# BienLuky/Rectified-SpaAttn

Hardware: AMD Instinct MI355X
Metric: attention-layer TFLOPs/sec (rectified block-sparse attention, HunyuanVideo seq~120k d=128 bf16) (higher is better)
Workload: dtype bf16; 1 GPU; hunyuan_720p_128f: B=1 H=24 S=115456 (115200 visual + 256 text, 200 valid) D=128, top_k=90, regime=r2 (p_remain=0.0, neighbors=none); heads_per_gpu=24, parallelism=head-shard x1, world_size=1

## Files before the change

### include/rsa.h

```cpp
#ifndef RSA_H_
#define RSA_H_

#include <stddef.h>
#include <stdint.h>

#ifdef __cplusplus
extern "C" {
#endif

#define RSA_BLOCK 128

typedef enum rsa_status {
    RSA_OK = 0,
    RSA_ERR_BAD_ARG = -1,
    RSA_ERR_UNSUPPORTED = -2,
    RSA_ERR_WORKSPACE = -3,
    RSA_ERR_LAUNCH = -4
} rsa_status;

typedef enum rsa_dtype { RSA_BF16 = 0, RSA_FP16 = 1 } rsa_dtype;

typedef struct rsa_layout {
    int32_t B, H, D;
    int32_t S;
// ... 50 lines not shown

int rsa_buffer_bytes(const rsa_layout* lay, size_t sizes[RSA_NUM_BUFFERS], size_t* total);

int rsa_carve_workspace(const rsa_layout* lay, void* ws, size_t ws_bytes, rsa_buffers* out);

int rsa_pool_stats(const rsa_layout* lay, rsa_tensor4 q, rsa_tensor4 k, rsa_tensor4 v, const rsa_buffers* buf,
                   void* stream);

int rsa_pooled_scores(const rsa_layout* lay, rsa_tensor4 k, const rsa_buffers* buf, void* stream);

int rsa_select_mask(const rsa_layout* lay, const uint8_t* neighbor, int top_k, float p_remain,
                    const rsa_buffers* buf, void* stream);

int rsa_compensation(const rsa_layout* lay, const rsa_buffers* buf, void* stream);

int rsa_block_sparse_fwd(const rsa_layout* lay, rsa_tensor4 q, rsa_tensor4 k, rsa_tensor4 v,
                         const rsa_buffers* buf, rsa_out4 out, void* stream);

int rsa_rectified_attention(const rsa_layout* lay, rsa_tensor4 q, rsa_tensor4 k, rsa_tensor4 v,
                            const uint8_t* neighbor, int top_k, float p_remain, void* workspace,
                            size_t workspace_bytes, rsa_out4 out, void* stream);

int rsa_dense_fwd(int B, int H, int Sq, int Sk, int D, int dtype, rsa_tensor4 q, rsa_tensor4 k, rsa_tensor4 v,
                  int q_split, int kv_split, rsa_out4 out, void* stream);
int rsa_dense_causal_fwd(int B, int H, int Sq, int Sk, int D, int dtype, rsa_tensor4 q, rsa_tensor4 k, rsa_tensor4 v,
                         int q_split, int kv_split, rsa_out4 out, void* stream);

#define RSA_MASK_BOOL 1
#define RSA_MASK_ADD_2BYTE 2
#define RSA_MASK_ADD_F32 3
// ... 7 lines not shown
                          uint64_t seed, rsa_out4 out, void* stream);

typedef struct rsa_layout_ex {
    rsa_layout base;
    int32_t block;
    int32_t reserved[3];
} rsa_layout_ex;
int rsa_buffer_bytes_ex(const rsa_layout_ex* lay, size_t sizes[RSA_NUM_BUFFERS], size_t* total);
int rsa_carve_workspace_ex(const rsa_layout_ex* lay, void* ws, size_t ws_bytes, rsa_buffers* out);
int rsa_pool_stats_ex(const rsa_layout_ex* lay, rsa_tensor4 q, rsa_tensor4 k, rsa_tensor4 v, const rsa_buffers* buf,
                      void* stream);
int rsa_pooled_scores_ex(const rsa_layout_ex* lay, rsa_tensor4 k, const rsa_buffers* buf, void* stream);
int rsa_select_mask_ex(const rsa_layout_ex* lay, const uint8_t* neighbor, int top_k, float p_remain,
                       const rsa_buffers* buf, void* stream);
int rsa_compensation_ex(const rsa_layout_ex* lay, const rsa_buffers* buf, void* stream);
int rsa_block_sparse_fwd_ex(const rsa_layout_ex* lay, rsa_tensor4 q, rsa_tensor4 k, rsa_tensor4 v,
                            const rsa_buffers* buf, rsa_out4 out, void* stream);
int rsa_rectified_attention_ex(const rsa_layout_ex* lay, rsa_tensor4 q, rsa_tensor4 k, rsa_tensor4 v,
                               const uint8_t* neighbor, int top_k, float p_remain, void* workspace,
                               size_t workspace_bytes, rsa_out4 out, void* stream);

int rsa_block_mask_to_lists(int B, int H, int NQ, int NK, const uint8_t* mask, int64_t mask_stride_b, int64_t mask_stride_h,
                            int64_t mask_stride_q, uint32_t* bitmask, int32_t* cols, int32_t* counts, void* stream);
int rsa_lists_to_block_mask(int B, int H, int NQ, int NK, const uint32_t* bitmask, uint8_t* mask, void* stream);

int rsa_block_sparse_plain_fwd(int B, int H, int Sq, int Sk, int D, int dtype, int block, int NQ, int NK, int kv_valid,
                               double sm_scale, rsa_tensor4 q, rsa_tensor4 k, rsa_tensor4 v, const int32_t* cols,
                               const int32_t* counts, float* tpart, size_t tpart_bytes, rsa_out4 out, void* stream);

int rsa_select_from_mask(const rsa_layout* lay, const uint8_t* mask, int64_t mask_stride_b, int64_t mask_stride_h,
// ... 110 lines not shown
```

### rectified_spaattn_amd/_core.py

```python
from __future__ import annotations

import ctypes
import math
from dataclasses import dataclass
from typing import Dict, Optional

import torch

from . import _lib
from ._lib import BLOCK, BUFFER_NAMES, RsaBuffers, RsaFp8Operands, RsaLayout, RsaLayoutEx, RsaOut4, RsaTensor4


def check_block(block: int) -> int:
    if block not in _lib.BLOCKS:
        raise NotImplementedError(f"the HIP path is built for block_size_M = block_size_N in {_lib.BLOCKS}, got {block}")
    return int(block)


@dataclass
class LayoutSpec:
    S: int
    NB_total: int
    NBv: int
    n_txt: int
# ... 304 lines not shown
        cb, st = ctypes.byref(self.cb), _stream()
        tk = self.t[1]
        (k2, lay), (k4, _) = self._fn("rsa_pooled_scores"), self._fn("rsa_compensation")
        with torch.cuda.device(self.q.device):
            _lib.check(k2(lay, tk, cb, st), "rsa_pooled_scores")
            if self.mask is not None:
                k3m, _ = self._fn("rsa_select_from_mask")
                _lib.check(k3m(lay, self.mask.data_ptr(), *self.mask_strides, cb, st), "rsa_select_from_mask")
            else:
                k3, _ = self._fn("rsa_select_mask")
                _lib.check(k3(lay, self.nbr.data_ptr() if self.nbr is not None else None, self.top_k,
                              self.p, cb, st), "rsa_select_mask")
            _lib.check(k4(lay, cb, st), "rsa_compensation")

    def select(self):
        self.select_pool()
        self.select_rest()

    def attend(self):
        tq, tk, tv = self.t
        if self.fp8 is not None and self.fp8_pv:
            with torch.cuda.device(self.q.device):
                _lib.check(self.L.rsa_block_sparse_fwd_fp8pv(ctypes.byref(self.lay), tq, tk, ctypes.byref(self.cf),
                                                             ctypes.byref(self.cb), self.o4, _stream()),
                           "rsa_block_sparse_fwd_fp8pv")
            return self.out
        if self.fp8 is not None:
            with torch.cuda.device(self.q.device):
                _lib.check(self.L.rsa_block_sparse_fwd_fp8(ctypes.byref(self.lay), ctypes.byref(self.cf),
                                                           ctypes.byref(self.cb), self.o4, _stream()),
                           "rsa_block_sparse_fwd_fp8")
            return self.out
# ... 199 lines not shown
```

### rectified_spaattn_amd/_lib.py

```python
from __future__ import annotations

import ctypes
import os

import torch

_HERE = os.path.dirname(os.path.abspath(__file__))
LIB_PATH = os.path.join(_HERE, "librsa_hip.so")

RSA_BF16, RSA_FP16 = 0, 1
BLOCK = 128
BLOCKS = (64, 128)
HEADER_VERSION = 601


class RsaError(RuntimeError):
    pass


class RsaLayout(ctypes.Structure):
    _fields_ = [(n, ctypes.c_int32) for n in (
        "B", "H", "D", "S", "NB_total", "NBv", "n_txt", "kv_valid", "pool_valid", "text_end_block",
        "first_frame_blocks", "q_text_valid", "kv_text_valid", "dtype")]

# ... 61 lines not shown
    L.rsa_qk_layernorm_rope.restype = i32
    L.rsa_norm_rope_heads.argtypes = [i32, i32, i32, i32, i32, vp, i64, i64, vp, f32, i32, i32, vp, vp, RsaOut4, vp]
    L.rsa_norm_rope_heads.restype = i32
    L.rsa_rel_l1.argtypes = [vp, vp, i64, i32, vp, vp, vp]
    L.rsa_rel_l1.restype = i32
    L.rsa_set_tuning.argtypes = [ctypes.c_char_p, i32]
    L.rsa_set_tuning.restype = i32
    L.rsa_set_shard_invariant.argtypes = [i32]
    L.rsa_set_shard_invariant.restype = i32
    L.rsa_buffer_bytes.argtypes = [P(RsaLayout), P(sz * NUM_BUFFERS), P(sz)]
    L.rsa_carve_workspace.argtypes = [P(RsaLayout), vp, sz, P(RsaBuffers)]
    L.rsa_pool_stats.argtypes = [P(RsaLayout), RsaTensor4, RsaTensor4, RsaTensor4, P(RsaBuffers), vp]
    L.rsa_pooled_scores.argtypes = [P(RsaLayout), RsaTensor4, P(RsaBuffers), vp]
    L.rsa_select_mask.argtypes = [P(RsaLayout), vp, i32, f32, P(RsaBuffers), vp]
    L.rsa_compensation.argtypes = [P(RsaLayout), P(RsaBuffers), vp]
    L.rsa_block_sparse_fwd.argtypes = [P(RsaLayout), RsaTensor4, RsaTensor4, RsaTensor4, P(RsaBuffers), RsaOut4, vp]
    L.rsa_rectified_attention.argtypes = [P(RsaLayout), RsaTensor4, RsaTensor4, RsaTensor4, vp, i32, f32, vp, sz,
                                          RsaOut4, vp]
    L.rsa_buffer_bytes_ex.argtypes = [P(RsaLayoutEx), P(sz * NUM_BUFFERS), P(sz)]
    L.rsa_carve_workspace_ex.argtypes = [P(RsaLayoutEx), vp, sz, P(RsaBuffers)]
    L.rsa_pool_stats_ex.argtypes = [P(RsaLayoutEx), RsaTensor4, RsaTensor4, RsaTensor4, P(RsaBuffers), vp]
    L.rsa_pooled_scores_ex.argtypes = [P(RsaLayoutEx), RsaTensor4, P(RsaBuffers), vp]
    L.rsa_select_mask_ex.argtypes = [P(RsaLayoutEx), vp, i32, f32, P(RsaBuffers), vp]
    L.rsa_compensation_ex.argtypes = [P(RsaLayoutEx), P(RsaBuffers), vp]
    L.rsa_block_sparse_fwd_ex.argtypes = [P(RsaLayoutEx), RsaTensor4, RsaTensor4, RsaTensor4, P(RsaBuffers), RsaOut4, vp]
    L.rsa_rectified_attention_ex.argtypes = [P(RsaLayoutEx), RsaTensor4, RsaTensor4, RsaTensor4, vp, i32, f32, vp, sz,
                                             RsaOut4, vp]
    L.rsa_estimate_pr_gain_ex.argtypes = [i32] * 6 + [vp] * 9
    L.rsa_block_mask_to_lists.argtypes = [i32] * 4 + [vp, i64, i64, i64, vp, vp, vp, vp]
    L.rsa_lists_to_block_mask.argtypes = [i32] * 4 + [vp, vp, vp]
# ... 50 lines not shown
    L.rsa_ipc_close.argtypes = [vp]
    for name in ("rsa_comm_unique_id", "rsa_comm_create", "rsa_comm_destroy", "rsa_comm_count", "rsa_allgather_heads",
                 "rsa_allgather_heads_p2p", "rsa_ipc_export", "rsa_ipc_open", "rsa_ipc_close", "rsa_ipc_offset",
                 "rsa_p2p_state_alloc", "rsa_p2p_state_free", "rsa_p2p_state_timeout"):
        getattr(L, name).restype = i32
    for name in ("rsa_fp8_operand_bytes", "rsa_carve_fp8_operands", "rsa_quantize_fp8", "rsa_block_sparse_fwd_fp8",
                 "rsa_rectified_attention_fp8", "rsa_rectified_attention_fp8pv", "rsa_pool_stats_fp8", "rsa_dense_fp8_bytes",
                 "rsa_dense_fwd_fp8"):
        getattr(L, name).restype = i32
    for name in ("rsa_buffer_bytes", "rsa_carve_workspace", "rsa_pool_stats", "rsa_pooled_scores",
                 "rsa_select_mask", "rsa_compensation", "rsa_block_sparse_fwd", "rsa_rectified_attention",
                 "rsa_dense_fwd", "rsa_dense_masked_fwd", "rsa_estimate_pr_gain", "rsa_buffer_bytes_ex", "rsa_carve_workspace_ex",
                 "rsa_pool_stats_ex", "rsa_pooled_scores_ex", "rsa_select_mask_ex", "rsa_compensation_ex", "rsa_block_sparse_fwd_ex",
                 "rsa_rectified_attention_ex", "rsa_estimate_pr_gain_ex"):
        getattr(L, name).restype = i32
    for key in ("k5_tsplit", "k3_prefix", "k3_long", "k4_split", "k5_rows256", "k5_static", "k5_w64", "k5_gsync", "k5_gsync_ratio", "k5_text_last", "k5_tail_split"):
        val = os.environ.get("RSA_" + key.upper())
        if val is not None:
            check_rc = L.rsa_set_tuning(key.encode(), int(val))
            if check_rc != 0:
                raise RsaError(f"RSA_{key.upper()} is set but rsa_set_tuning refused it (export RSA_TUNING=1)")
    _lib = L
    return L


EXPORTED = ("rsa_version", "rsa_abi_check", "rsa_buffer_bytes", "rsa_carve_workspace", "rsa_pool_stats", "rsa_pooled_scores",
            "rsa_select_mask", "rsa_compensation", "rsa_block_sparse_fwd", "rsa_rectified_attention",
            "rsa_dense_fwd", "rsa_dense_causal_fwd", "rsa_dense_masked_fwd", "rsa_dense_dropout_fwd", "rsa_estimate_pr_gain", "rsa_status_string", "rsa_last_hip_error", "rsa_set_tuning", "rsa_set_shard_invariant", "rsa_gilbert_mapping",
            "rsa_gilbert_block_neighbors", "rsa_permute_tokens", "rsa_qk_norm_rope", "rsa_qk_layernorm_rope", "rsa_norm_rope_heads", "rsa_fp8_operand_bytes",
            "rsa_carve_fp8_operands", "rsa_quantize_fp8", "rsa_block_sparse_fwd_fp8", "rsa_block_sparse_fwd_fp8pv", "rsa_rectified_attention_fp8", "rsa_rectified_attention_fp8pv",
            "rsa_pool_stats_fp8", "rsa_dense_fp8_bytes", "rsa_dense_fwd_fp8", "rsa_dense_causal_fwd_fp8", "rsa_dense_fwd_fp8pv", "rsa_rel_l1",
            "rsa_comm_unique_id", "rsa_comm_create", "rsa_comm_destroy", "rsa_comm_count", "rsa_allgather_heads",
            "rsa_allgather_heads_p2p", "rsa_p2p_state_bytes", "rsa_p2p_state_alloc", "rsa_p2p_state_free", "rsa_p2p_state_timeout", "rsa_ipc_export", "rsa_ipc_open", "rsa_ipc_close",
            "rsa_ipc_offset", "rsa_buffer_bytes_ex", "rsa_carve_workspace_ex", "rsa_pool_stats_ex", "rsa_pooled_scores_ex",
            "rsa_select_mask_ex", "rsa_compensation_ex", "rsa_block_sparse_fwd_ex", "rsa_rectified_attention_ex", "rsa_estimate_pr_gain_ex",
            "rsa_block_mask_to_lists", "rsa_lists_to_block_mask", "rsa_block_sparse_plain_fwd", "rsa_select_from_mask",
            "rsa_select_from_mask_ex", "rsa_rectified_attention_masked", "rsa_rectified_attention_masked_ex")


def check(status: int, what: str):
    if status == 0:
        return
    msg = f"{what}: {lib().rsa_status_string(status).decode()} (rsa_status {status})"
    if status == -4:
        msg += f": {lib().rsa_last_hip_error().decode()}"
    if status == -2:
        raise AssertionError(msg)
    raise RsaError(msg)
```

### rectified_spaattn_amd/csrc/rsa_attn.hip

```cpp
#include <stdlib.h>

#include <atomic>
#include <mutex>
#include "rsa_attn.h"

static int g_k5_tsplit = 1;
extern int g_rsa_k3_prefix;
extern int g_rsa_k3_long;
extern int g_rsa_k4_split;
extern int g_rsa_k2_dma;
static int g_k5_tail_split = 1;
static int g_k5_text_last = 1;
static int g_shard_invariant = 0;
static int g_k5_gsync_ratio = 2;
int rsa_gsync_ratio() { return g_k5_gsync_ratio; }
static int g_k5_rows256 = 1;
static int g_k5_static = 1;
int rsa_k5_static() { return g_k5_static; }
static int g_k5_gsync = 1;

static int g_k5_w64 = 3;
static bool k5_runs_w64(int D, int blk) { return blk == RSA_BLOCK && ((D == 128 && (g_k5_w64 & 1)) || (D == 64 && (g_k5_w64 & 2))); }

extern "C" int rsa_set_tuning(const char* key, int value) {
    static const bool enabled = [] { const char* e = getenv("RSA_TUNING"); return e && e[0] == '1'; }();
    if (!key) return RSA_ERR_BAD_ARG;
    if (!enabled) return RSA_ERR_UNSUPPORTED;
    if (strcmp(key, "k3_prefix") == 0) { g_rsa_k3_prefix = value; return RSA_OK; }
    if (strcmp(key, "k3_long") == 0) { g_rsa_k3_long = value; return RSA_OK; }
    if (strcmp(key, "k4_split") == 0) { g_rsa_k4_split = value; return RSA_OK; }
    if (strcmp(key, "k2_dma") == 0) { g_rsa_k2_dma = value; return RSA_OK; }
    if (strcmp(key, "k5_static") == 0) { g_k5_static = value; return RSA_OK; }
    if (strcmp(key, "k5_rows256") == 0) { g_k5_rows256 = value; return RSA_OK; }
    if (strcmp(key, "k5_tsplit") == 0) { g_k5_tsplit = value; return RSA_OK; }
    if (strcmp(key, "k5_w64") == 0) { g_k5_w64 = value; return RSA_OK; }
    if (strcmp(key, "k5_gsync") == 0) { g_k5_gsync = value; return RSA_OK; }
    if (strcmp(key, "k5_gsync_ratio") == 0) { g_k5_gsync_ratio = value; return RSA_OK; }
    if (strcmp(key, "k5_text_last") == 0) { g_k5_text_last = value; return RSA_OK; }
    if (strcmp(key, "k5_tail_split") == 0) { g_k5_tail_split = value; return RSA_OK; }
    if (strcmp(key, "fp8_variant") == 0) { rsa_set_fp8_variant(value); return RSA_OK; }
    if (strcmp(key, "fp8_smooth_k") == 0) { rsa_set_fp8_smooth_k(value); return RSA_OK; }
    return RSA_ERR_BAD_ARG;
}

template <typename Tag>
__global__ __launch_bounds__(256) void text_combine_kernel(const float* __restrict__ tpart, unsigned short* out,
// ... 329 lines not shown
                             rsa_tensor4 v, int q_split, int kv_split, rsa_out4 out, void* stream) {
    return dense_fwd(B, H, Sq, Sk, D, dtype, q, k, v, q_split, kv_split, 0, out, stream);
}

extern "C" int rsa_dense_causal_fwd(int B, int H, int Sq, int Sk, int D, int dtype, rsa_tensor4 q, rsa_tensor4 k,
                                    rsa_tensor4 v, int q_split, int kv_split, rsa_out4 out, void* stream) {
    return dense_fwd(B, H, Sq, Sk, D, dtype, q, k, v, q_split, kv_split, 1, out, stream);
}

extern "C" int rsa_rectified_attention(const rsa_layout* l, rsa_tensor4 q, rsa_tensor4 k, rsa_tensor4 v,
                                       const uint8_t* neighbor, int top_k, float p_remain, void* workspace,
                                       size_t workspace_bytes, rsa_out4 out, void* stream) {
    rsa_buffers buf;
    int st = rsa_carve_workspace(l, workspace, workspace_bytes, &buf);
    if (st != RSA_OK) return st;
    if ((st = rsa_pool_stats(l, q, k, v, &buf, stream))) return st;
    if ((st = rsa_pooled_scores(l, k, &buf, stream))) return st;
    if ((st = rsa_select_mask(l, neighbor, top_k, p_remain, &buf, stream))) return st;
    if ((st = rsa_compensation(l, &buf, stream))) return st;
    return rsa_block_sparse_fwd(l, q, k, v, &buf, out, stream);
}

extern "C" int rsa_rectified_attention_ex(const rsa_layout_ex* lx, rsa_tensor4 q, rsa_tensor4 k, rsa_tensor4 v,
                                          const uint8_t* neighbor, int top_k, float p_remain, void* workspace,
                                          size_t workspace_bytes, rsa_out4 out, void* stream) {
    if (!rsa_layout_ex_ok(lx)) return RSA_ERR_BAD_ARG;
    if (lx->block == RSA_BLOCK)
        return rsa_rectified_attention(&lx->base, q, k, v, neighbor, top_k, p_remain, workspace, workspace_bytes, out, stream);
    rsa_buffers buf;
    int st = rsa_carve_workspace_ex(lx, workspace, workspace_bytes, &buf);
    if (st != RSA_OK) return st;
    if ((st = rsa_pool_stats_ex(lx, q, k, v, &buf, stream))) return st;
    if ((st = rsa_pooled_scores_ex(lx, k, &buf, stream))) return st;
    if ((st = rsa_select_mask_ex(lx, neighbor, top_k, p_remain, &buf, stream))) return st;
    if ((st = rsa_compensation_ex(lx, &buf, stream))) return st;
    return rsa_block_sparse_fwd_ex(lx, q, k, v, &buf, out, stream);
}
```

### rectified_spaattn_amd/csrc/rsa_stats.hip

```cpp
#include "rsa_common.h"
#include "rsa_fp8_emit.h"

struct PoolArgs {
    const unsigned short* src[3];
    long sb[3], sh[3], ss[3];
    float* mean[3];
    float* mad[3];
    const float* ext_mean[3];
    int nblk[3];
    int valid[3];
    int H;
    int BH, NB_total;
    Fp8Emit f8;
};

template <int D, typename Tag, bool F8, int BLK = RSA_BLOCK>
__global__ __launch_bounds__(D * 2) void pool_stats_kernel(PoolArgs a) {
    constexpr int NI = BLK / 16;
    constexpr int CH = D / 8;
    constexpr int NTH = 16 * CH;
    constexpr int NW = NTH / 64;
    const int which = F8 ? (int)(blockIdx.x % 3) : (int)blockIdx.z;
    const int blk = F8 ? (int)(blockIdx.x / 3) : (int)blockIdx.x;
    if (blk >= a.nblk[which]) return;
// ... 88 lines not shown
            for (int e = 0; e < 8; ++e) {
                float tot;
                if (NW == 4)
                    tot = (red[0][c * 8 + e] + red[1][c * 8 + e]) +
                          (red[2 % NW][c * 8 + e] + red[3 % NW][c * 8 + e]);
                else
                    tot = red[0][c * 8 + e] + red[1][c * 8 + e];
                r[e] = tot * (1.0f / BLK);
            }
            float4* o = reinterpret_cast<float4*>(a.mad[which] + orow);
            o[0] = make_float4(r[0], r[1], r[2], r[3]);
            o[1] = make_float4(r[4], r[5], r[6], r[7]);
        }
    }
    emit_f8();
}

struct ScoreArgs {
    const float *qbar, *aq, *kbar, *ak;
    const unsigned short* ktxt;
    long ksb, ksh, kss;
    float* scores;
    uint8_t* unrel;
    int NBv, n_txt, NS, D, H, BH;
    int txt0;
};

typedef float k2_f32x16 __attribute__((ext_vector_type(16)));
__device__ __forceinline__ int ncols_of(const ScoreArgs& a, int mode) { return mode == 0 ? a.NBv : a.n_txt; }

// ... 302 lines not shown
            } else if (pos >= len) {
                dl = true;
            }
        }
        c = __shfl(cl, ln, 64);
        count += __shfl(cnt, ln, 64);
        done = __shfl((int)dl, ln, 64) != 0;
        over = __shfl((int)ol, ln, 64) != 0;
    }
    passed = over;
    return count;
}

#define RSA_SEL_CAP 256

template <int KPL, int PASS>
__global__ __launch_bounds__(256) void select_mask_kernel(SelectArgs a) {
    extern __shared__ __attribute__((aligned(16))) unsigned char smem[];
    const int lane = threadIdx.x & 63, wv = threadIdx.x >> 6;
    const long row = (long)blockIdx.x * 4 + wv;
    if (row >= a.rows_total) return;
    if constexpr (PASS == 1) {
        if (a.counts[row] != -1) return;
    }
    const int qblk = (int)(row % a.NBv);
    unsigned char* base = smem + (size_t)wv * a.lds_per_wave;
    float* et = reinterpret_cast<float*>(base);
    float* pr = et + a.et_len;
    uint8_t* kept = reinterpret_cast<uint8_t*>(pr + ((a.L + 3) & ~3));
    const float* sc = a.scores + row * a.NS;
    const bool has_txt = a.n_txt > 0;

    constexpr int NE = KPL + 8;
    float xv[NE];
    uint8_t urv[KPL], nbv[KPL];
// ... 563 lines not shown
    out->vbar = (float*)ptrs[4]; out->scores = (float*)ptrs[5]; out->unrel = (uint8_t*)ptrs[6];
    out->probs = (float*)ptrs[7]; out->w = (float*)ptrs[8]; out->R = (float*)ptrs[9]; out->comp = (float*)ptrs[10];
    out->bitmask = (uint32_t*)ptrs[11]; out->cols = (int32_t*)ptrs[12]; out->counts = (int32_t*)ptrs[13];
    out->tpart = (float*)ptrs[14];
    out->tpart_bytes = sizes[14];
    return RSA_OK;
}
extern "C" int rsa_carve_workspace(const rsa_layout* l, void* ws, size_t ws_bytes, rsa_buffers* out) {
    return carve_workspace_b(l, RSA_BLOCK, ws, ws_bytes, out);
}
extern "C" int rsa_carve_workspace_ex(const rsa_layout_ex* lx, void* ws, size_t ws_bytes, rsa_buffers* out) {
    return rsa_layout_ex_ok(lx) ? carve_workspace_b(&lx->base, lx->block, ws, ws_bytes, out) : RSA_ERR_BAD_ARG;
}

static int pool_stats_b(const rsa_layout* l, int blk, rsa_tensor4 q, rsa_tensor4 k, rsa_tensor4 v, const rsa_buffers* buf,
                        const Fp8Emit* f8, void* stream) {
    int st = rsa_check_layout_b(l, blk);
    if (st != RSA_OK) return st;
    if (!buf || !buf->qbar || !buf->aq || !buf->kbar || !buf->ak || !buf->vbar) return RSA_ERR_BAD_ARG;
    if ((st = rsa_check_tensor(q)) || (st = rsa_check_tensor(k)) || (st = rsa_check_tensor(v))) return st;
    PoolArgs a;
    const rsa_tensor4* ts[3] = {&q, &k, &v};
    for (int i = 0; i < 3; ++i) {
        a.src[i] = static_cast<const unsigned short*>(ts[i]->ptr);
        a.sb[i] = ts[i]->stride_b; a.sh[i] = ts[i]->stride_h; a.ss[i] = ts[i]->stride_s;
        a.ext_mean[i] = nullptr;
    }
    if (f8 != nullptr && blk != RSA_BLOCK) return RSA_ERR_UNSUPPORTED;
    const int vis_tok = l->NBv * blk;
    a.mean[0] = buf->qbar; a.mad[0] = buf->aq; a.nblk[0] = l->NBv; a.valid[0] = l->S < vis_tok ? l->S : vis_tok;
    a.mean[1] = buf->kbar; a.mad[1] = buf->ak; a.nblk[1] = l->NBv;
    a.valid[1] = l->pool_valid < vis_tok ? l->pool_valid : vis_tok;
    a.mean[2] = buf->vbar; a.mad[2] = nullptr; a.nblk[2] = l->NB_total; a.valid[2] = l->pool_valid;
    a.H = l->H;
    a.BH = l->B * l->H; a.NB_total = l->NB_total;
    dim3 grid(l->NB_total, l->B * l->H, 3);
    hipStream_t s = static_cast<hipStream_t>(stream);
    if (f8 != nullptr) {
        a.f8 = *f8;
        const dim3 grid8(3 * l->NB_total, l->B * l->H, 1);
        if (l->D == 128) {
            if (l->dtype == RSA_BF16) pool_stats_kernel<128, bf16_tag, true><<<grid8, 256, 0, s>>>(a);
            else pool_stats_kernel<128, fp16_tag, true><<<grid8, 256, 0, s>>>(a);
        } else {
            if (l->dtype == RSA_BF16) pool_stats_kernel<64, bf16_tag, true><<<grid8, 128, 0, s>>>(a);
            else pool_stats_kernel<64, fp16_tag, true><<<grid8, 128, 0, s>>>(a);
        }
        return rsa_launch_status();
    }
    if (blk == 64) {
        if (l->D == 128) {
// ... 55 lines not shown
        else pooled_scores_kernel<fp16_tag, 16><<<g0, 256, 0, s>>>(a);
    } else {
        if (l->dtype == RSA_BF16) pooled_scores_kernel<bf16_tag, 0><<<g0, 256, 0, s>>>(a);
        else pooled_scores_kernel<fp16_tag, 0><<<g0, 256, 0, s>>>(a);
    }
    return rsa_launch_status();
}

extern "C" int rsa_pooled_scores(const rsa_layout* l, rsa_tensor4 k, const rsa_buffers* buf, void* stream) {
    return pooled_scores_b(l, RSA_BLOCK, k, buf, stream);
}
extern "C" int rsa_pooled_scores_ex(const rsa_layout_ex* lx, rsa_tensor4 k, const rsa_buffers* buf, void* stream) {
    return rsa_layout_ex_ok(lx) ? pooled_scores_b(&lx->base, lx->block, k, buf, stream) : RSA_ERR_BAD_ARG;
}

static int select_mask_b(const rsa_layout* l, int blk, const uint8_t* neighbor, int top_k, float p_remain,
                         const rsa_buffers* buf, void* stream) {
    int st = rsa_check_layout_b(l, blk);
    if (st != RSA_OK) return st;
    if (!buf || !buf->scores || !buf->unrel || !buf->probs || !buf->w || !buf->R || !buf->bitmask || !buf->cols ||
        !buf->counts || top_k < 0)
        return RSA_ERR_BAD_ARG;
    if (l->NBv == 0) return RSA_OK;
    SelectArgs a;
    a.scores = buf->scores; a.unrel = buf->unrel; a.neighbor = neighbor;
    a.probs = buf->probs; a.w = buf->w; a.R = buf->R; a.bitmask = buf->bitmask; a.cols = buf->cols;
    a.counts = buf->counts;
    a.NBv = l->NBv; a.n_txt = l->n_txt; a.NS = l->NBv + l->n_txt; a.L = l->NBv + (l->n_txt > 0 ? 1 : 0);
    int n2 = 64;
    while (n2 < a.L) n2 <<= 1;
    a.N2 = n2; a.NB_total = l->NB_total; a.NW = (l->NB_total + 31) / 32;
    a.text_end_block = l->text_end_block; a.ffb = l->first_frame_blocks; a.top_k = top_k;
    a.thr = p_remain;
    a.blk = (float)blk;
    a.scale = (float)(1.0 / sqrt((double)l->D));
    a.rows_total = l->B * l->H * l->NBv;
    a.use_prefix = g_rsa_k3_prefix;
    a.et_len = (a.n_txt + 3) & ~3;
    if (a.et_len < 2 * RSA_SEL_CAP) a.et_len = 2 * RSA_SEL_CAP;
    const size_t per_wave = (((size_t)a.et_len * 4 + (size_t)((a.L + 3) & ~3) * 4 + (size_t)((a.NB_total + 7) & ~7)) + 15) &
                            ~(size_t)15;
    a.lds_per_wave = (int)per_wave;
    const size_t lds = per_wave * 4;
    hipStream_t s = static_cast<hipStream_t>(stream);
    if (g_rsa_k3_long || lds > 64 * 1024 || n2 > 4096 || a.NB_total > n2 + 63) {
        if (n2 > 8192 || a.NB_total > 8192) return RSA_ERR_UNSUPPORTED;
        const size_t lds_long = (((size_t)a.NS * 4 + 15) & ~(size_t)15) + (size_t)n2 * 8 + (((size_t)a.NB_total + 15) & ~(size_t)15);
        if (lds_long > 150 * 1024) return RSA_ERR_UNSUPPORTED;
        (void)hipFuncSetAttribute(reinterpret_cast<const void*>(select_mask_long_kernel), hipFuncAttributeMaxDynamicSharedMemorySize, (int)lds_long);
        (void)hipGetLastError();
        select_mask_long_kernel<<<dim3((unsigned)a.rows_total), 256, lds_long, s>>>(a);
        return rsa_launch_status();
    }
    dim3 grid((unsigned)((a.rows_total + 3) / 4));
    const int need = top_k > RSA_SEL_CAP / 2 ? top_k : RSA_SEL_CAP / 2;
    const bool two_pass = a.use_prefix && n2 / 64 > RSA_SEL_CAP / 64 && need <= RSA_SEL_CAP && a.L > RSA_SEL_CAP;
#define RSA_K3(K) \
    do { \
        if (two_pass) { \
            select_mask_kernel<K, 0><<<grid, 256, lds, s>>>(a); \
            select_mask_kernel<K, 1><<<grid, 256, lds, s>>>(a); \
        } else { \
            select_mask_kernel<K, 2><<<grid, 256, lds, s>>>(a); \
        } \
    } while (0)
    switch (n2 / 64) {
        case 1: select_mask_kernel<1, 2><<<grid, 256, lds, s>>>(a); break;
        case 2: select_mask_kernel<2, 2><<<grid, 256, lds, s>>>(a); break;
        case 4: select_mask_kernel<4, 2><<<grid, 256, lds, s>>>(a); break;
        case 8: RSA_K3(8); break;
        case 16: RSA_K3(16); break;
        case 32: RSA_K3(32); break;
        default: RSA_K3(64); break;
    }
#undef RSA_K3
    st = rsa_launch_status();
    if (st != RSA_OK) return st;
    return st;
}
extern "C" int rsa_select_mask(const rsa_layout* l, const uint8_t* neighbor, int top_k, float p_remain,
                               const rsa_buffers* buf, void* stream) {
    return select_mask_b(l, RSA_BLOCK, neighbor, top_k, p_remain, buf, stream);
}
extern "C" int rsa_select_mask_ex(const rsa_layout_ex* lx, const uint8_t* neighbor, int top_k, float p_remain,
// ... 11 lines not shown
    dim3 grid((l->NBv + 31) / 32, l->B * l->H);
    if (g_rsa_k4_split == 2 || (g_rsa_k4_split == 1 && (long)grid.x * grid.y >= 512)) {
        if (l->D == 128) compensation_split_kernel<128><<<grid, 256, 0, s>>>(buf->w, buf->vbar, buf->comp, l->NBv, L, l->NB_total);
        else compensation_split_kernel<64><<<grid, 128, 0, s>>>(buf->w, buf->vbar, buf->comp, l->NBv, L, l->NB_total);
        return rsa_launch_status();
    }
    if (l->D == 128) compensation_kernel<128><<<grid, 256, 0, s>>>(buf->w, buf->vbar, buf->comp, l->NBv, L, l->NB_total);
    else compensation_kernel<64><<<grid, 128, 0, s>>>(buf->w, buf->vbar, buf->comp, l->NBv, L, l->NB_total);
    return rsa_launch_status();
}
extern "C" int rsa_compensation(const rsa_layout* l, const rsa_buffers* buf, void* stream) {
    return compensation_b(l, RSA_BLOCK, buf, stream);
}
extern "C" int rsa_compensation_ex(const rsa_layout_ex* lx, const rsa_buffers* buf, void* stream) {
    return rsa_layout_ex_ok(lx) ? compensation_b(&lx->base, lx->block, buf, stream) : RSA_ERR_BAD_ARG;
}

extern "C" int rsa_estimate_pr_gain_ex(int BH, int NQ, int NK, int D, int dtype, int block, const void* q_blocks,
                                       const void* k_blocks, const float* q_pools, const float* k_pools,
                                       const float* scores, float* scratch_aq, float* scratch_ak, uint8_t* mask_out,
                                       void* stream) {
    if (block != 64 && block != RSA_BLOCK) return RSA_ERR_UNSUPPORTED;
    if (BH <= 0 || NQ <= 0 || NK <= 0 || !q_blocks || !k_blocks || !q_pools || !k_pools || !scores || !scratch_aq ||
        !scratch_ak || !mask_out)
        return RSA_ERR_BAD_ARG;
    if (D != 64 && D != 128) return RSA_ERR_UNSUPPORTED;
    if (dtype != RSA_BF16 && dtype != RSA_FP16) return RSA_ERR_UNSUPPORTED;
    hipStream_t s = static_cast<hipStream_t>(stream);
    for (int which = 0; which < 2; ++which) {
        PoolArgs a;
// ... 61 lines not shown
```

Baseline: 1181 TFLOP/s.

## Overlap V-block mean pooling with first select-mask pass in a mixed grid

```diff
diff --git a/include/rsa.h b/include/rsa.h
--- a/include/rsa.h
+++ b/include/rsa.h
@@ -88,6 +88,10 @@
 
 int rsa_compensation(const rsa_layout* lay, const rsa_buffers* buf, void* stream);
 
+int rsa_select_pass(const rsa_layout* lay, rsa_tensor4 q, rsa_tensor4 k, rsa_tensor4 v, const uint8_t* neighbor, int top_k,
+                    float p_remain, const rsa_buffers* buf, void* stream);
+int rsa_mix_map(unsigned n_main, unsigned n_pool, unsigned block_id, int* kind, unsigned* index);
+
 int rsa_block_sparse_fwd(const rsa_layout* lay, rsa_tensor4 q, rsa_tensor4 k, rsa_tensor4 v,
                          const rsa_buffers* buf, rsa_out4 out, void* stream);
 
@@ -125,6 +129,8 @@
 int rsa_select_mask_ex(const rsa_layout_ex* lay, const uint8_t* neighbor, int top_k, float p_remain,
                        const rsa_buffers* buf, void* stream);
 int rsa_compensation_ex(const rsa_layout_ex* lay, const rsa_buffers* buf, void* stream);
+int rsa_select_pass_ex(const rsa_layout_ex* lay, rsa_tensor4 q, rsa_tensor4 k, rsa_tensor4 v, const uint8_t* neighbor, int top_k,
+                       float p_remain, const rsa_buffers* buf, void* stream);
 int rsa_block_sparse_fwd_ex(const rsa_layout_ex* lay, rsa_tensor4 q, rsa_tensor4 k, rsa_tensor4 v,
                             const rsa_buffers* buf, rsa_out4 out, void* stream);
 int rsa_rectified_attention_ex(const rsa_layout_ex* lay, rsa_tensor4 q, rsa_tensor4 k, rsa_tensor4 v,
diff --git a/rectified_spaattn_amd/_core.py b/rectified_spaattn_amd/_core.py
--- a/rectified_spaattn_amd/_core.py
+++ b/rectified_spaattn_amd/_core.py
@@ -342,8 +342,15 @@
             _lib.check(k4(lay, cb, st), "rsa_compensation")
 
     def select(self):
-        self.select_pool()
-        self.select_rest()
+        if self.fp8 is not None or self.mask is not None:
+            self.select_pool()
+            self.select_rest()
+            return
+        fn, lay = self._fn("rsa_select_pass")
+        tq, tk, tv = self.t
+        with torch.cuda.device(self.q.device):
+            _lib.check(fn(lay, tq, tk, tv, self.nbr.data_ptr() if self.nbr is not None else None, self.top_k, self.p,
+                          ctypes.byref(self.cb), _stream()), "rsa_select_pass")
 
     def attend(self):
         tq, tk, tv = self.t
diff --git a/rectified_spaattn_amd/_lib.py b/rectified_spaattn_amd/_lib.py
--- a/rectified_spaattn_amd/_lib.py
+++ b/rectified_spaattn_amd/_lib.py
@@ -99,6 +99,11 @@
     L.rsa_pooled_scores.argtypes = [P(RsaLayout), RsaTensor4, P(RsaBuffers), vp]
     L.rsa_select_mask.argtypes = [P(RsaLayout), vp, i32, f32, P(RsaBuffers), vp]
     L.rsa_compensation.argtypes = [P(RsaLayout), P(RsaBuffers), vp]
+    L.rsa_select_pass.argtypes = [P(RsaLayout), RsaTensor4, RsaTensor4, RsaTensor4, vp, i32, f32, P(RsaBuffers), vp]
+    L.rsa_select_pass_ex.argtypes = [P(RsaLayoutEx), RsaTensor4, RsaTensor4, RsaTensor4, vp, i32, f32, P(RsaBuffers), vp]
+    L.rsa_mix_map.argtypes = [ctypes.c_uint, ctypes.c_uint, ctypes.c_uint, P(i32), P(ctypes.c_uint)]
+    for name in ("rsa_select_pass", "rsa_select_pass_ex", "rsa_mix_map"):
+        getattr(L, name).restype = i32
     L.rsa_block_sparse_fwd.argtypes = [P(RsaLayout), RsaTensor4, RsaTensor4, RsaTensor4, P(RsaBuffers), RsaOut4, vp]
     L.rsa_rectified_attention.argtypes = [P(RsaLayout), RsaTensor4, RsaTensor4, RsaTensor4, vp, i32, f32, vp, sz,
                                           RsaOut4, vp]
@@ -179,7 +184,7 @@
                  "rsa_pool_stats_ex", "rsa_pooled_scores_ex", "rsa_select_mask_ex", "rsa_compensation_ex", "rsa_block_sparse_fwd_ex",
                  "rsa_rectified_attention_ex", "rsa_estimate_pr_gain_ex"):
         getattr(L, name).restype = i32
-    for key in ("k5_tsplit", "k3_prefix", "k3_long", "k4_split", "k5_rows256", "k5_static", "k5_w64", "k5_gsync", "k5_gsync_ratio", "k5_text_last", "k5_tail_split"):
+    for key in ("k5_tsplit", "k3_prefix", "k3_long", "k4_split", "select_overlap", "k5_rows256", "k5_static", "k5_w64", "k5_gsync", "k5_gsync_ratio", "k5_text_last", "k5_tail_split"):
         val = os.environ.get("RSA_" + key.upper())
         if val is not None:
             check_rc = L.rsa_set_tuning(key.encode(), int(val))
@@ -200,7 +205,8 @@
             "rsa_ipc_offset", "rsa_buffer_bytes_ex", "rsa_carve_workspace_ex", "rsa_pool_stats_ex", "rsa_pooled_scores_ex",
             "rsa_select_mask_ex", "rsa_compensation_ex", "rsa_block_sparse_fwd_ex", "rsa_rectified_attention_ex", "rsa_estimate_pr_gain_ex",
             "rsa_block_mask_to_lists", "rsa_lists_to_block_mask", "rsa_block_sparse_plain_fwd", "rsa_select_from_mask",
-            "rsa_select_from_mask_ex", "rsa_rectified_attention_masked", "rsa_rectified_attention_masked_ex")
+            "rsa_select_from_mask_ex", "rsa_rectified_attention_masked", "rsa_rectified_attention_masked_ex",
+            "rsa_select_pass", "rsa_select_pass_ex", "rsa_mix_map")
 
 
 def check(status: int, what: str):
diff --git a/rectified_spaattn_amd/csrc/rsa_attn.hip b/rectified_spaattn_amd/csrc/rsa_attn.hip
--- a/rectified_spaattn_amd/csrc/rsa_attn.hip
+++ b/rectified_spaattn_amd/csrc/rsa_attn.hip
@@ -9,6 +9,7 @@
 extern int g_rsa_k3_long;
 extern int g_rsa_k4_split;
 extern int g_rsa_k2_dma;
+extern int g_rsa_select_overlap;
 static int g_k5_tail_split = 1;
 static int g_k5_text_last = 1;
 static int g_shard_invariant = 0;
@@ -30,6 +31,7 @@
     if (strcmp(key, "k3_long") == 0) { g_rsa_k3_long = value; return RSA_OK; }
     if (strcmp(key, "k4_split") == 0) { g_rsa_k4_split = value; return RSA_OK; }
     if (strcmp(key, "k2_dma") == 0) { g_rsa_k2_dma = value; return RSA_OK; }
+    if (strcmp(key, "select_overlap") == 0) { g_rsa_select_overlap = value; return RSA_OK; }
     if (strcmp(key, "k5_static") == 0) { g_k5_static = value; return RSA_OK; }
     if (strcmp(key, "k5_rows256") == 0) { g_k5_rows256 = value; return RSA_OK; }
     if (strcmp(key, "k5_tsplit") == 0) { g_k5_tsplit = value; return RSA_OK; }
@@ -389,10 +391,7 @@
     rsa_buffers buf;
     int st = rsa_carve_workspace(l, workspace, workspace_bytes, &buf);
     if (st != RSA_OK) return st;
-    if ((st = rsa_pool_stats(l, q, k, v, &buf, stream))) return st;
-    if ((st = rsa_pooled_scores(l, k, &buf, stream))) return st;
-    if ((st = rsa_select_mask(l, neighbor, top_k, p_remain, &buf, stream))) return st;
-    if ((st = rsa_compensation(l, &buf, stream))) return st;
+    if ((st = rsa_select_pass(l, q, k, v, neighbor, top_k, p_remain, &buf, stream))) return st;
     return rsa_block_sparse_fwd(l, q, k, v, &buf, out, stream);
 }
 
@@ -405,9 +404,6 @@
     rsa_buffers buf;
     int st = rsa_carve_workspace_ex(lx, workspace, workspace_bytes, &buf);
     if (st != RSA_OK) return st;
-    if ((st = rsa_pool_stats_ex(lx, q, k, v, &buf, stream))) return st;
-    if ((st = rsa_pooled_scores_ex(lx, k, &buf, stream))) return st;
-    if ((st = rsa_select_mask_ex(lx, neighbor, top_k, p_remain, &buf, stream))) return st;
-    if ((st = rsa_compensation_ex(lx, &buf, stream))) return st;
+    if ((st = rsa_select_pass_ex(lx, q, k, v, neighbor, top_k, p_remain, &buf, stream))) return st;
     return rsa_block_sparse_fwd_ex(lx, q, k, v, &buf, out, stream);
 }
diff --git a/rectified_spaattn_amd/csrc/rsa_stats.hip b/rectified_spaattn_amd/csrc/rsa_stats.hip
--- a/rectified_spaattn_amd/csrc/rsa_stats.hip
+++ b/rectified_spaattn_amd/csrc/rsa_stats.hip
@@ -1,5 +1,6 @@
 #include "rsa_common.h"
 #include "rsa_fp8_emit.h"
+#include <type_traits>
 
 struct PoolArgs {
     const unsigned short* src[3];
@@ -126,6 +127,60 @@
         }
     }
     emit_f8();
+}
+
+typedef unsigned pool_u32x4 __attribute__((ext_vector_type(4)));
+template <int D, typename Tag, int BLK>
+__device__ __forceinline__ void pool_mean_block(const unsigned short* src, long sb, long sh, long ss, int valid, int nblk, float* omean,
+                                                int H, int blk, int bh, float (*red)[D]) {
+    constexpr int NI = BLK / 16, CH = D / 8, NW = D * 2 / 64;
+    const int b = bh / H, h = bh % H;
+    const int t = threadIdx.x;
+    const int c = t % CH, g = t / CH;
+    const unsigned short* base = src + (long)b * sb + (long)h * sh + c * 8;
+    uint4 raw[NI];
+#pragma unroll
+    for (int i = 0; i < NI; ++i) {
+        const int row = blk * BLK + 16 * i + g;
+        raw[i] = make_uint4(0, 0, 0, 0);
+        if (row < valid) {
+            const pool_u32x4 r4 = __builtin_nontemporal_load(reinterpret_cast<const pool_u32x4*>(base + (long)row * ss));
+            raw[i] = make_uint4(r4[0], r4[1], r4[2], r4[3]);
+        }
+    }
+    float s[8];
+#pragma unroll
+    for (int i = 0; i < NI; ++i) {
+        const unsigned w[4] = {raw[i].x, raw[i].y, raw[i].z, raw[i].w};
+#pragma unroll
+        for (int e = 0; e < 4; ++e) {
+            const float x0 = rsa_to_f32<Tag>((unsigned short)(w[e] & 0xFFFF)), x1 = rsa_to_f32<Tag>((unsigned short)(w[e] >> 16));
+            s[2 * e] = i == 0 ? x0 : s[2 * e] + x0;
+            s[2 * e + 1] = i == 0 ? x1 : s[2 * e + 1] + x1;
+        }
+    }
+#pragma unroll
+    for (int m = CH; m < 64; m <<= 1)
+#pragma unroll
+        for (int e = 0; e < 8; ++e) s[e] = s[e] + __shfl_xor(s[e], m, 64);
+    if ((t & 63) < CH)
+#pragma unroll
+        for (int e = 0; e < 8; ++e) red[t >> 6][c * 8 + e] = s[e];
+    __syncthreads();
+    if (g != 0) return;
+    float mean[8];
+#pragma unroll
+    for (int e = 0; e < 8; ++e) {
+        float tot;
+        if (NW == 4)
+            tot = (red[0][c * 8 + e] + red[1][c * 8 + e]) + (red[2 % NW][c * 8 + e] + red[3 % NW][c * 8 + e]);
+        else
+            tot = red[0][c * 8 + e] + red[1][c * 8 + e];
+        mean[e] = tot * (1.0f / BLK);
+    }
+    float4* o = reinterpret_cast<float4*>(omean + ((long)bh * nblk + blk) * D + c * 8);
+    o[0] = make_float4(mean[0], mean[1], mean[2], mean[3]);
+    o[1] = make_float4(mean[4], mean[5], mean[6], mean[7]);
 }
 
 struct ScoreArgs {
@@ -458,11 +513,45 @@
 
 #define RSA_SEL_CAP 256
 
-template <int KPL, int PASS>
-__global__ __launch_bounds__(256) void select_mask_kernel(SelectArgs a) {
+__host__ __device__ __forceinline__ void rsa_mix_slot(unsigned b, unsigned n_main, unsigned n_pool, int* kind, unsigned* idx) {
+    const unsigned long long n = (unsigned long long)n_main + n_pool;
+    const unsigned lo = (unsigned)((unsigned long long)b * n_pool / n), hi = (unsigned)(((unsigned long long)b + 1) * n_pool / n);
+    *kind = hi > lo;
+    *idx = hi > lo ? lo : b - lo;
+}
+extern "C" int rsa_mix_map(unsigned n_main, unsigned n_pool, unsigned block_id, int* kind, unsigned* index) {
+    if (!kind || !index || (unsigned long long)n_main + n_pool > 0xFFFFFFFFull || block_id >= n_main + n_pool) return RSA_ERR_BAD_ARG;
+    rsa_mix_slot(block_id, n_main, n_pool, kind, index);
+    return RSA_OK;
+}
+template <typename PTag> struct PoolRide {
+    const unsigned short* src;
+    long sb, sh, ss;
+    float* mean;
+    int valid, nblk, H;
+    unsigned n_main, n_pool;
+    explicit PoolRide(const PoolArgs& p, unsigned nm, unsigned np)
+        : src(p.src[2]), sb(p.sb[2]), sh(p.sh[2]), ss(p.ss[2]), mean(p.mean[2]), valid(p.valid[2]), nblk(p.nblk[2]), H(p.H), n_main(nm), n_pool(np) {}
+};
+template <> struct PoolRide<void> {};
+
+
+template <int KPL, int PASS, typename PTag = void>
+__global__ __launch_bounds__(256) void select_mask_kernel(SelectArgs a, PoolRide<PTag> ride) {
     extern __shared__ __attribute__((aligned(16))) unsigned char smem[];
+    unsigned wg = blockIdx.x;
+    if constexpr (!std::is_void<PTag>::value) {
+        int kind;
+        rsa_mix_slot(blockIdx.x, ride.n_main, ride.n_pool, &kind, &wg);
+        if (kind) {
+            pool_mean_block<128, PTag, RSA_BLOCK>(ride.src, ride.sb, ride.sh, ride.ss, ride.valid, ride.nblk, ride.mean, ride.H,
+                                                  (int)(wg % (unsigned)ride.nblk), (int)(wg / (unsigned)ride.nblk),
+                                                  reinterpret_cast<float (*)[128]>(smem));
+            return;
+        }
+    }
     const int lane = threadIdx.x & 63, wv = threadIdx.x >> 6;
-    const long row = (long)blockIdx.x * 4 + wv;
+    const long row = (long)wg * 4 + wv;
     if (row >= a.rows_total) return;
     if constexpr (PASS == 1) {
         if (a.counts[row] != -1) return;
@@ -1056,12 +1145,13 @@
 }
 
 static int pool_stats_b(const rsa_layout* l, int blk, rsa_tensor4 q, rsa_tensor4 k, rsa_tensor4 v, const rsa_buffers* buf,
-                        const Fp8Emit* f8, void* stream) {
+                        const Fp8Emit* f8, void* stream, int nz = 3, PoolArgs* out = nullptr) {
     int st = rsa_check_layout_b(l, blk);
     if (st != RSA_OK) return st;
     if (!buf || !buf->qbar || !buf->aq || !buf->kbar || !buf->ak || !buf->vbar) return RSA_ERR_BAD_ARG;
     if ((st = rsa_check_tensor(q)) || (st = rsa_check_tensor(k)) || (st = rsa_check_tensor(v))) return st;
     PoolArgs a;
+    a.f8 = Fp8Emit{};
     const rsa_tensor4* ts[3] = {&q, &k, &v};
     for (int i = 0; i < 3; ++i) {
         a.src[i] = static_cast<const unsigned short*>(ts[i]->ptr);
@@ -1076,7 +1166,8 @@
     a.mean[2] = buf->vbar; a.mad[2] = nullptr; a.nblk[2] = l->NB_total; a.valid[2] = l->pool_valid;
     a.H = l->H;
     a.BH = l->B * l->H; a.NB_total = l->NB_total;
-    dim3 grid(l->NB_total, l->B * l->H, 3);
+    if (out) *out = a;
+    dim3 grid(l->NB_total, l->B * l->H, nz);
     hipStream_t s = static_cast<hipStream_t>(stream);
     if (f8 != nullptr) {
         a.f8 = *f8;
@@ -1162,8 +1253,24 @@
     return rsa_layout_ex_ok(lx) ? pooled_scores_b(&lx->base, lx->block, k, buf, stream) : RSA_ERR_BAD_ARG;
 }
 
+struct K3Form { int L, n2, et_len; size_t per_wave, lds; bool long_form, two_pass; };
+static K3Form k3_form(const rsa_layout* l, int top_k) {
+    K3Form f;
+    f.L = l->NBv + (l->n_txt > 0 ? 1 : 0);
+    f.n2 = 64;
+    while (f.n2 < f.L) f.n2 <<= 1;
+    f.et_len = (l->n_txt + 3) & ~3;
+    if (f.et_len < 2 * RSA_SEL_CAP) f.et_len = 2 * RSA_SEL_CAP;
+    f.per_wave = (((size_t)f.et_len * 4 + (size_t)((f.L + 3) & ~3) * 4 + (size_t)((l->NB_total + 7) & ~7)) + 15) & ~(size_t)15;
+    f.lds = f.per_wave * 4;
+    f.long_form = g_rsa_k3_long || f.lds > 64 * 1024 || f.n2 > 4096 || l->NB_total > f.n2 + 63;
+    const int need = top_k > RSA_SEL_CAP / 2 ? top_k : RSA_SEL_CAP / 2;
+    f.two_pass = !f.long_form && g_rsa_k3_prefix && f.n2 / 64 > RSA_SEL_CAP / 64 && need <= RSA_SEL_CAP && f.L > RSA_SEL_CAP;
+    return f;
+}
+
 static int select_mask_b(const rsa_layout* l, int blk, const uint8_t* neighbor, int top_k, float p_remain,
-                         const rsa_buffers* buf, void* stream) {
+                         const rsa_buffers* buf, void* stream, const PoolArgs* vpool = nullptr) {
     int st = rsa_check_layout_b(l, blk);
     if (st != RSA_OK) return st;
     if (!buf || !buf->scores || !buf->unrel || !buf->probs || !buf->w || !buf->R || !buf->bitmask || !buf->cols ||
@@ -1174,9 +1281,9 @@
     a.scores = buf->scores; a.unrel = buf->unrel; a.neighbor = neighbor;
     a.probs = buf->probs; a.w = buf->w; a.R = buf->R; a.bitmask = buf->bitmask; a.cols = buf->cols;
     a.counts = buf->counts;
-    a.NBv = l->NBv; a.n_txt = l->n_txt; a.NS = l->NBv + l->n_txt; a.L = l->NBv + (l->n_txt > 0 ? 1 : 0);
-    int n2 = 64;
-    while (n2 < a.L) n2 <<= 1;
+    const K3Form f = k3_form(l, top_k);
+    const int n2 = f.n2;
+    a.NBv = l->NBv; a.n_txt = l->n_txt; a.NS = l->NBv + l->n_txt; a.L = f.L;
     a.N2 = n2; a.NB_total = l->NB_total; a.NW = (l->NB_total + 31) / 32;
     a.text_end_block = l->text_end_block; a.ffb = l->first_frame_blocks; a.top_k = top_k;
     a.thr = p_remain;
@@ -1184,14 +1291,12 @@
     a.scale = (float)(1.0 / sqrt((double)l->D));
     a.rows_total = l->B * l->H * l->NBv;
     a.use_prefix = g_rsa_k3_prefix;
-    a.et_len = (a.n_txt + 3) & ~3;
-    if (a.et_len < 2 * RSA_SEL_CAP) a.et_len = 2 * RSA_SEL_CAP;
-    const size_t per_wave = (((size_t)a.et_len * 4 + (size_t)((a.L + 3) & ~3) * 4 + (size_t)((a.NB_total + 7) & ~7)) + 15) &
-                            ~(size_t)15;
-    a.lds_per_wave = (int)per_wave;
-    const size_t lds = per_wave * 4;
+    a.et_len = f.et_len;
+    a.lds_per_wave = (int)f.per_wave;
+    const size_t lds = f.lds;
     hipStream_t s = static_cast<hipStream_t>(stream);
-    if (g_rsa_k3_long || lds > 64 * 1024 || n2 > 4096 || a.NB_total > n2 + 63) {
+    if (vpool != nullptr && (!f.two_pass || l->D != 128 || blk != RSA_BLOCK)) return RSA_ERR_BAD_ARG;
+    if (f.long_form) {
         if (n2 > 8192 || a.NB_total > 8192) return RSA_ERR_UNSUPPORTED;
         const size_t lds_long = (((size_t)a.NS * 4 + 15) & ~(size_t)15) + (size_t)n2 * 8 + (((size_t)a.NB_total + 15) & ~(size_t)15);
         if (lds_long > 150 * 1024) return RSA_ERR_UNSUPPORTED;
@@ -1201,21 +1306,38 @@
         return rsa_launch_status();
     }
     dim3 grid((unsigned)((a.rows_total + 3) / 4));
-    const int need = top_k > RSA_SEL_CAP / 2 ? top_k : RSA_SEL_CAP / 2;
-    const bool two_pass = a.use_prefix && n2 / 64 > RSA_SEL_CAP / 64 && need <= RSA_SEL_CAP && a.L > RSA_SEL_CAP;
+    const bool two_pass = f.two_pass;
+    if (vpool != nullptr) {
+        const unsigned n_main = grid.x, n_pool = (unsigned)l->NB_total * (unsigned)(l->B * l->H);
+        const dim3 gm(n_main + n_pool);
+#define RSA_K3P(K) \
+        do { \
+            if (l->dtype == RSA_BF16) select_mask_kernel<K, 0, bf16_tag><<<gm, 256, lds, s>>>(a, PoolRide<bf16_tag>(*vpool, n_main, n_pool)); \
+            else select_mask_kernel<K, 0, fp16_tag><<<gm, 256, lds, s>>>(a, PoolRide<fp16_tag>(*vpool, n_main, n_pool)); \
+            select_mask_kernel<K, 1><<<grid, 256, lds, s>>>(a, PoolRide<void>{}); \
+        } while (0)
+        switch (n2 / 64) {
+            case 8: RSA_K3P(8); break;
+            case 16: RSA_K3P(16); break;
+            case 32: RSA_K3P(32); break;
+            default: RSA_K3P(64); break;
+        }
+#undef RSA_K3P
+        return rsa_launch_status();
+    }
 #define RSA_K3(K) \
     do { \
         if (two_pass) { \
-            select_mask_kernel<K, 0><<<grid, 256, lds, s>>>(a); \
-            select_mask_kernel<K, 1><<<grid, 256, lds, s>>>(a); \
+            select_mask_kernel<K, 0><<<grid, 256, lds, s>>>(a, PoolRide<void>{}); \
+            select_mask_kernel<K, 1><<<grid, 256, lds, s>>>(a, PoolRide<void>{}); \
         } else { \
-            select_mask_kernel<K, 2><<<grid, 256, lds, s>>>(a); \
+            select_mask_kernel<K, 2><<<grid, 256, lds, s>>>(a, PoolRide<void>{}); \
         } \
     } while (0)
     switch (n2 / 64) {
-        case 1: select_mask_kernel<1, 2><<<grid, 256, lds, s>>>(a); break;
-        case 2: select_mask_kernel<2, 2><<<grid, 256, lds, s>>>(a); break;
-        case 4: select_mask_kernel<4, 2><<<grid, 256, lds, s>>>(a); break;
+        case 1: select_mask_kernel<1, 2><<<grid, 256, lds, s>>>(a, PoolRide<void>{}); break;
+        case 2: select_mask_kernel<2, 2><<<grid, 256, lds, s>>>(a, PoolRide<void>{}); break;
+        case 4: select_mask_kernel<4, 2><<<grid, 256, lds, s>>>(a, PoolRide<void>{}); break;
         case 8: RSA_K3(8); break;
         case 16: RSA_K3(16); break;
         case 32: RSA_K3(32); break;
@@ -1257,6 +1379,39 @@
 }
 extern "C" int rsa_compensation_ex(const rsa_layout_ex* lx, const rsa_buffers* buf, void* stream) {
     return rsa_layout_ex_ok(lx) ? compensation_b(&lx->base, lx->block, buf, stream) : RSA_ERR_BAD_ARG;
+}
+
+int g_rsa_select_overlap = 1;
+#define RSA_OVERLAP_MIN_WG (256 * 6)
+static int select_pass_b(const rsa_layout* l, int blk, rsa_tensor4 q, rsa_tensor4 k, rsa_tensor4 v, const uint8_t* neighbor,
+                         int top_k, float p_remain, const rsa_buffers* buf, void* stream) {
+    int st = rsa_check_layout_b(l, blk);
+    if (st != RSA_OK) return st;
+    if (!buf || !buf->qbar || !buf->aq || !buf->kbar || !buf->ak || !buf->vbar || !buf->scores || !buf->unrel || !buf->probs ||
+        !buf->w || !buf->R || !buf->bitmask || !buf->cols || !buf->counts || !buf->comp || top_k < 0)
+        return RSA_ERR_BAD_ARG;
+    if ((st = rsa_check_tensor(q)) || (st = rsa_check_tensor(k)) || (st = rsa_check_tensor(v))) return st;
+    const K3Form f = k3_form(l, top_k);
+    if (l->NBv > 0 && f.long_form) {
+        const size_t lds_long = (((size_t)(l->NBv + l->n_txt) * 4 + 15) & ~(size_t)15) + (size_t)f.n2 * 8 + (((size_t)l->NB_total + 15) & ~(size_t)15);
+        if (f.n2 > 8192 || l->NB_total > 8192 || lds_long > 150 * 1024) return RSA_ERR_UNSUPPORTED;
+    }
+    const long n_pool = (long)l->NB_total * l->B * l->H, n_main = ((long)l->B * l->H * l->NBv + 3) / 4;
+    const bool can = blk == RSA_BLOCK && l->D == 128 && l->NBv > 0 && f.two_pass && n_pool + n_main < (1L << 31);
+    const bool overlap = can && (g_rsa_select_overlap == 2 || (g_rsa_select_overlap == 1 && n_main > RSA_OVERLAP_MIN_WG));
+    PoolArgs pa;
+    if ((st = pool_stats_b(l, blk, q, k, v, buf, nullptr, stream, overlap ? 2 : 3, &pa))) return st;
+    if ((st = pooled_scores_b(l, blk, k, buf, stream))) return st;
+    if ((st = select_mask_b(l, blk, neighbor, top_k, p_remain, buf, stream, overlap ? &pa : nullptr))) return st;
+    return compensation_b(l, blk, buf, stream);
+}
+extern "C" int rsa_select_pass(const rsa_layout* l, rsa_tensor4 q, rsa_tensor4 k, rsa_tensor4 v, const uint8_t* neighbor,
+                               int top_k, float p_remain, const rsa_buffers* buf, void* stream) {
+    return select_pass_b(l, RSA_BLOCK, q, k, v, neighbor, top_k, p_remain, buf, stream);
+}
+extern "C" int rsa_select_pass_ex(const rsa_layout_ex* lx, rsa_tensor4 q, rsa_tensor4 k, rsa_tensor4 v, const uint8_t* neighbor,
+                                  int top_k, float p_remain, const rsa_buffers* buf, void* stream) {
+    return rsa_layout_ex_ok(lx) ? select_pass_b(&lx->base, lx->block, q, k, v, neighbor, top_k, p_remain, buf, stream) : RSA_ERR_BAD_ARG;
 }
 
 extern "C" int rsa_estimate_pr_gain_ex(int BH, int NQ, int NK, int D, int dtype, int block, const void* q_blocks,
```

Measured after the change: 1184 TFLOP/s, median of 2. Within noise of the previous version (+0.2%).
